# bee-hive/MedGP

Hardware: AMD Instinct MI355X
Metric: per-patient nlml+grad evals/sec at D=24 N=512 (higher is better)
Workload: dtype f64; 1 GPU; config 4 shard: 512 patients/GPU x N=512, D=24, Q=5, R=8, H=1114, LMC-SM + hier-gamma prior, nlml+grad; patients_per_gpu=512, cohort=512, N=512, D=24, Q=5, R=8, H=1114, parallelism=patient-sharded x1 (no collective)

## Files before the change

medgp_amd/csrc/kernels_wgrad.h:

```cpp
#pragma once
#include "medgp_dev.h"
#include "kernels_assemble.h"

#define WG_KC 32
#define WG_THREADS 256
#ifndef WG_MINWAVES
#define WG_MINWAVES 3
#endif

#define WG_CHUNK_MFMA(ac, buf) \
    _Pragma("unroll") for (int h = 0; h < 4; h++) \
        _Pragma("unroll") for (int ct = 0; ct < 4; ct++) { \
            if (ct > ctmax) continue;    \
            const v2d bf = *(const v2d *)&Bs[buf][16 * ct + li][8 * h + 2 * g]; \
            _Pragma("unroll") for (int s = 0; s < 2; s++) acc[ct] = __builtin_amdgcn_mfma_f64_16x16x4f64(ac[h][s], bf[s], acc[ct], 0, 0, 0); \
        }

template <int QT, int Q0 = 0, int PF = 1>
__global__ void __launch_bounds__(WG_THREADS, WG_MINWAVES) k_wgrad(MedgpDev L, int nbatch, int ntiles, int nbp) {
    __shared__ __attribute__((aligned(16))) double smem[2 * 64 * (WG_KC + 2)];
    typedef double (*BsT)[64][WG_KC + 2];
    BsT Bs = (BsT)smem;
    double (*Ws)[66] = (double (*)[66])smem;
    __shared__ __attribute__((aligned(16))) double rowc[4][16][2 + 2 * QT];

    int b, tix;
    if (nbatch >= 64) {
        const int xcd = blockIdx.x & 7, rest = blockIdx.x >> 3;
        b = (rest / ntiles) * 8 + xcd;
        tix = rest % ntiles;
    } else {
        int x = blockIdx.x;
        const int total = nbp * ntiles;
        if (x >= total) return;
        if (PF > 1 && total <= 1024 && ((x >> 8) & 1)) {
            const int v0 = x & ~255, m = min(256, total - v0);
            x = v0 + (m - 1 - (x & 255));
        }
        b = x % nbp;
        tix = x / nbp;
    }
    if (b >= nbatch) return;
    if (L.status[b] < 0) return;
    const int slot = __builtin_amdgcn_readfirstlane(L.bslot[b]);
    const int n = __builtin_amdgcn_readfirstlane(L.pn[slot]);
    const int ld = L.ldn, npad = medgp_roundup(n, 64), nb = npad / 64;
    int I, J;
    tile_decode(tix, I, J);
    if (I >= nb) return;
    const int tid = threadIdx.x, lane = tid & 63, li = lane & 15, g = lane >> 4;
    const int w = __builtin_amdgcn_readfirstlane(tid >> 6);
    const double *U = L.Linv + (size_t)b * ld * ld;

#ifdef MEDGP_STAMPS
    unsigned long long wst[4] = {0, 0, 0, 0}, wlast;
    asm volatile("s_memtime %0\n\ts_waitcnt lgkmcnt(0)" : "=s"(wlast)::"memory");
#define WSTAMP(k) do { unsigned long long t_; asm volatile("s_memtime %0\n\ts_waitcnt lgkmcnt(0)" : "=s"(t_)::"memory"); wst[k] += t_ - wlast; wlast = t_; } while (0)
#else
#define WSTAMP(k) do {} while (0)
#endif
    v4d acc[4];
#pragma unroll
    for (int ct = 0; ct < 4; ct++) acc[ct] = (v4d){0.0, 0.0, 0.0, 0.0};
    {
        const int k0 = 64 * I, nch = (npad - k0) / WG_KC;
        const int ctmax = (I == J) ? w : 3;
        const double *Arow = U + (size_t)(64 * I + 16 * w + li) * ld + k0 + 2 * g;
        const int srow = tid >> 2, scg = (tid & 3) * 8;
        const double *Bsrc = U + (size_t)(64 * J + srow) * ld + k0 + scg;
        if constexpr (PF == 1) {
            v2d bst[4], an[4];
#pragma unroll
            for (int u = 0; u < 4; u++) bst[u] = *(const v2d *)(Bsrc + 2 * u);
#pragma unroll
            for (int h = 0; h < 4; h++) an[h] = *(const v2d *)(Arow + 8 * h);
#pragma unroll
            for (int u = 0; u < 4; u++) *(v2d *)&Bs[0][srow][scg + 2 * u] = bst[u];
            __syncthreads();
            for (int c = 0; c < nch; c++) {
                const int buf = c & 1;
                v2d ac[4];
#pragma unroll
                for (int h = 0; h < 4; h++) ac[h] = an[h];
                if (c + 1 < nch) {
#pragma unroll
                    for (int u = 0; u < 4; u++) bst[u] = *(const v2d *)(Bsrc + (c + 1) * WG_KC + 2 * u);
#pragma unroll
                    for (int h = 0; h < 4; h++) an[h] = *(const v2d *)(Arow + (c + 1) * WG_KC + 8 * h);
                }
                WG_CHUNK_MFMA(ac, buf);
                if (c + 1 < nch) {
#pragma unroll
                    for (int u = 0; u < 4; u++) *(v2d *)&Bs[buf ^ 1][srow][scg + 2 * u] = bst[u];
                }
                __syncthreads();
            }
        } else {
            v2d bst[PF][4], an[PF][4];
#pragma unroll
            for (int st = 0; st < PF; st++)
                if (st < nch) {
#pragma unroll
                    for (int u = 0; u < 4; u++) bst[st][u] = *(const v2d *)(Bsrc + st * WG_KC + 2 * u);
#pragma unroll
                    for (int h = 0; h < 4; h++) an[st][h] = *(const v2d *)(Arow + st * WG_KC + 8 * h);
                }
#pragma unroll
            for (int u = 0; u < 4; u++) *(v2d *)&Bs[0][srow][scg + 2 * u] = bst[0][u];
            __syncthreads();
            for (int c0 = 0; c0 < nch; c0 += PF) {
#pragma unroll
                for (int st = 0; st < PF; st++) {
                    const int c = c0 + st;
                    if (c >= nch) break;
                    v2d ac[4];
#pragma unroll
                    for (int h = 0; h < 4; h++) ac[h] = an[st][h];
                    if (c + PF < nch) {
#pragma unroll
                        for (int u = 0; u < 4; u++) bst[st][u] = *(const v2d *)(Bsrc + (c + PF) * WG_KC + 2 * u);
#pragma unroll
                        for (int h = 0; h < 4; h++) an[st][h] = *(const v2d *)(Arow + (c + PF) * WG_KC + 8 * h);
                    }
                    WG_CHUNK_MFMA(ac, (st & 1));
                    if (c + 1 < nch) {
#pragma unroll
                        for (int u = 0; u < 4; u++) *(v2d *)&Bs[(st + 1) & 1][srow][scg + 2 * u] = bst[(st + 1) % PF][u];
                    }
                    __syncthreads();
                }
            }
        }
    }
    WSTAMP(0);
#pragma unroll
    for (int ct = 0; ct < 4; ct++)
#pragma unroll
        for (int r = 0; r < 4; r++) Ws[16 * w + 4 * r + g][16 * ct + li] = acc[ct][r];
    __syncthreads();

    WSTAMP(1);
    const double *hyp = L.hyp + (size_t)b * L.hyp_stride;
    const double *t = L.pt + (size_t)slot * L.pld;
    const int *meta = L.pmeta + (size_t)slot * L.pld;
    const double *alpha = L.alpha + (size_t)b * ld;
    const int *seg = L.pseg + (size_t)slot * (L.D + 1);
    const int *roff = L.proff + (size_t)slot * (L.D + 1), *coff = L.pcoff + (size_t)slot * (L.D + 1);
    const double *csb = L.cs + ((size_t)b * L.Q + Q0) * ld, *snb = L.sn + ((size_t)b * L.Q + Q0) * ld;
    double *slab = L.slab + (size_t)b * L.slab_stride;
    const int Qall = L.Q;
    const int Rmax = L.slab_R, Cmax = L.slab_C;

    double wq[QT], cq[QT];
#pragma unroll
    for (int q = 0; q < QT; q++) { wq[q] = hyp[hyp_off_w(L) + Q0 + q]; cq[q] = hyp[hyp_off_c(L) + Q0 + q]; }
    double cq2n[QT];
#pragma unroll
    for (int q = 0; q < QT; q++) cq2n[q] = uniform_d(-cq[q] * MEDGP_LOG2E);
    const int j = 64 * J + lane;
    const bool jv = j < n;
    const double tj = t[j], aj = alpha[j];
    const int mj = jv ? meta[j] : -1;
    double csj[QT], snj[QT];
#pragma unroll
    for (int q = 0; q < QT; q++) { csj[q] = csb[q * ld + j]; snj[q] = snb[q * ld + j]; }
    const int mprev = __shfl_up(mj, 1);
    const bool leader = (lane == 0) || (mj != mprev);
    const unsigned long long lmask = __ballot(leader);
    int segend;
    {
        unsigned long long above = (lane == 63) ? 0ull : (lmask >> (lane + 1));
        segend = above ? (lane + 1 + __builtin_ctzll(above)) : 64;
    }
    const unsigned long long upto = lmask & ((lane == 63) ? ~0ull : ((2ull << lane) - 1ull));
    const int segstart = 63 - __builtin_clzll(upto);
    const bool seglast = (lane == segend - 1);
    const int cslot = (mj >= 0) ? coff[mj] + (J - seg[mj] / 64) : 0;
    const int rg = 4 * I + w;

    double sS[QT], sM[QT], sV[QT];
#pragma unroll
    for (int q = 0; q < QT; q++) { sS[q] = 0.0; sM[q] = 0.0; sV[q] = 0.0; }
    int mcur = -2;
    const int irow = 64 * I + 16 * w + (lane & 15);
    const double r_t = t[irow], r_a = alpha[irow];
    const int r_m = (irow < n) ? meta[irow] : -1;
    double r_cs[QT], r_sn[QT];
#pragma unroll
    for (int q = 0; q < QT; q++) { r_cs[q] = csb[q * ld + irow]; r_sn[q] = snb[q * ld + irow]; }
    if (lane < 16) {
        rowc[w][lane][0] = r_t; rowc[w][lane][1] = r_a;
#pragma unroll
        for (int q = 0; q < QT; q++) { rowc[w][lane][2 + 2 * q] = r_cs[q]; rowc[w][lane][3 + 2 * q] = r_sn[q]; }
    }
    __builtin_amdgcn_wave_barrier();
    for (int rr = 0; rr <= 16; rr++) {
        const int i = 64 * I + 16 * w + rr;
        int mi = -1;
        if (rr < 16) mi = __builtin_amdgcn_readlane(r_m, rr);
        if (mi != mcur) {
            if (mcur >= 0) {
                const int rslot = roff[mcur] + (rg - seg[mcur] / 16);
                double fv[3 * QT];
#pragma unroll
                for (int q = 0; q < QT; q++) { fv[q] = sS[q]; fv[QT + q] = -wq[q] * sM[q]; fv[2 * QT + q] = -2.0 * cq[q] * sV[q]; }
#pragma unroll
                for (int dlt = 1; dlt < 64; dlt <<= 1) {
                    double up[3 * QT];
#pragma unroll
                    for (int k = 0; k < 3 * QT; k++) up[k] = __shfl_up(fv[k], dlt);
                    if (lane - dlt >= segstart) {
#pragma unroll
                        for (int k = 0; k < 3 * QT; k++) fv[k] += up[k];
                    }
                }
                if (seglast && mj >= 0) {
#pragma unroll
                    for (int k = 0; k < 3 * QT; k++) slab[((size_t)((k / QT) * Qall + Q0 + (k % QT)) * Rmax + rslot) * Cmax + cslot] = fv[k];
                }
            }
#pragma unroll
            for (int q = 0; q < QT; q++) { sS[q] = 0.0; sM[q] = 0.0; sV[q] = 0.0; }
            mcur = mi;
        }
        if (rr == 16 || mi < 0) continue;
        const v2d ta = *(const v2d *)&rowc[w][rr][0];
        const double ti = ta[0], ai = ta[1];
        double wv = Ws[16 * w + rr][lane] - ai * aj;
        if (I == J && j == i) L.wdiag[(size_t)b * ld + i] = wv;
        const bool valid = jv && (j <= i);
        wv = valid ? ((mi == mj && j < i) ? 2.0 * wv : wv) : 0.0;
        const double dt = ti - tj, dd = dt * dt;
#pragma unroll
        for (int q = 0; q < QT; q++) {
            const v2d csn = *(const v2d *)&rowc[w][rr][2 + 2 * q];
            const double ci = csn[0], si = csn[1];
            const double we = wv * exp2_nonpos(cq2n[q] * dd);
            const double cd = ci * csj[q] + si * snj[q];
            const double sd = si * csj[q] - ci * snj[q];
            const double p = we * cd;
            sS[q] += p;
            sM[q] += (we * sd) * dt;
            sV[q] += p * dd;
        }
    }
    WSTAMP(2);
#ifdef MEDGP_STAMPS
    if (lane == 0 && b < 64) {
        unsigned long long *dbg = (unsigned long long *)(L.xk + (size_t)b * 64 * 64);
        for (int e = 0; e < 3; e++) atomicAdd(&dbg[e], wst[e]);
        atomicAdd(&dbg[3], 1ull);
    }
#endif
}
```

medgp_amd/csrc/medgp_capi.hip:

```cpp
#include "../../include/medgp_hip.h"
#include "medgp_dev.h"
#include "kernels_core.h"
#include "kernels_v0.h"
#include "kernels_cholinv.h"
#include "kernels_cholinv_la.h"
#include "kernels_assemble.h"
#include "kernels_wgrad.h"
#include "kernels_io.h"
#include "kernels_cohort.h"

#include <algorithm>
#include <chrono>
#include <cmath>
#include <cstdarg>
#include <cstdio>
#include <cstdlib>
#include <cstring>
#include <string>
#include <vector>

namespace {

enum KernelId { KID_PREP = 0, KID_ASSEMBLE, KID_CHOLINV, KID_LA_STEP, KID_LA_AUX, KID_LAUUM, KID_GRADBINS, KID_WGRAD, KID_EPILOGUE, KID_PREDICT, KID_COUNT };
const char *const kKernelNames[KID_COUNT] = {"k_prep", "k_assemble", "k_cholinv", "k_la_step", "k_la_aux", "k_lauum", "k_gradbins", "k_wgrad", "k_epilogue", "k_predict"};
// ... 554 lines not shown
#endif
        if (route == ROUTE_WG44) hipLaunchKernelGGL((k_cholinv<4, 4, 0>), dim3(nbatch), dim3(256), 0, stream, L, want_mode);
        else hipLaunchKernelGGL((k_cholinv<8, 4, 0>), dim3(nbatch), dim3(512), 0, stream, L, want_mode);
    }
    int from_slab = 0;
#ifdef MEDGP_STAMPS
    if (getenv("MEDGP_DBG_NOWGRAD")) { HIPCHK(c, hipGetLastError()); return MEDGP_OK; }
#endif
    if (flag_grad) {
        const int wg_tiles = tri(nt64);
        const int nbp = (ragged && nbatch < 64) ? (nbatch | 1) : nbatch;
        const dim3 tg(std::max(8 * ((nbatch + 7) / 8), nbp) * wg_tiles), tb(WG_THREADS);
        from_slab = 1;
        Launcher lw(c, KID_WGRAD, stream);
        const int pf = c->wgrad_deep >= 0 ? c->wgrad_deep : ((long)nbatch * wg_tiles <= 16L * c->num_cu ? 2 : 1);
#define MEDGP_WGL(QQ, Q0) do { if (pf >= 2) hipLaunchKernelGGL((k_wgrad<QQ, Q0, 2>), tg, tb, 0, stream, L, nbatch, wg_tiles, nbp); \
                               else hipLaunchKernelGGL((k_wgrad<QQ, Q0, 1>), tg, tb, 0, stream, L, nbatch, wg_tiles, nbp); } while (0)
#define MEDGP_WG1(QQ) case QQ: MEDGP_WGL(QQ, 0); break;
#define MEDGP_WG2(QR) case 8 + QR: MEDGP_WGL(8, 0); MEDGP_WGL(QR, 8); break;
        switch (c->use_v0 ? 0 : L.Q) {
        MEDGP_WG1(1) MEDGP_WG1(2) MEDGP_WG1(3) MEDGP_WG1(4) MEDGP_WG1(5) MEDGP_WG1(6) MEDGP_WG1(7) MEDGP_WG1(8)
        MEDGP_WG2(1) MEDGP_WG2(2) MEDGP_WG2(3) MEDGP_WG2(4) MEDGP_WG2(5) MEDGP_WG2(6) MEDGP_WG2(7) MEDGP_WG2(8)
#undef MEDGP_WG1
#undef MEDGP_WG2
#undef MEDGP_WGL
        default: from_slab = 0; break;
        }
        if (!from_slab) lw.kid = -1;
        lw.finish();
        if (!from_slab) {
            { Launcher l(c, KID_LAUUM, stream); hipLaunchKernelGGL(k_lauum_v0, dim3(tri(nt64), nbatch), dim3(256), 0, stream, L); }
            const int nbins = L.Q * tri(L.D);
            { Launcher l(c, KID_GRADBINS, stream); hipLaunchKernelGGL(k_gradbins_v0, dim3((nbins + 255) / 256, nbatch), dim3(256), 0, stream, L); }
        }
    }
    if (flag_grad && from_slab) {
        const int nbins3 = 3 * L.Q * tri(L.D);
        Launcher l(c, KID_EPILOGUE, stream);
        hipLaunchKernelGGL(k_slabsum, dim3(nbatch, (nbins3 + 255) / 256), dim3(256), 0, stream, L);
    }
    if (nlml_dev) {
        Launcher l(c, KID_EPILOGUE, stream);
        const int nparts = (2 * nbatch >= c->num_cu) ? 1 : std::min(MEDGP_EPI_PARTS, (L.H + 255) / 256);
        hipLaunchKernelGGL(k_epilogue, dim3(nbatch, nparts), dim3(256), 0, stream, L, theta_dev, flag_grad, from_slab, nlml_dev, grad_dev, (int *)status_dev);
    }
    HIPCHK(c, hipGetLastError());
    return MEDGP_OK;
}


void choose_routes(const medgp_ctx *c, BatchPlan &P, std::vector<LaNeed> &las, std::vector<int> &la_of) {
    long long S = 0;
    for (const SizeClass &k : P.cls) S += k.tsum;
    las.clear();
    la_of.assign(P.cls.size(), -1);
    for (size_t i = 0; i < P.cls.size(); i++) {
        SizeClass &k = P.cls[i];
        bool la = false;
        if (!c->use_v0 && !c->pin_route && k.nbmax >= 2) {
            if (c->force_mc > 0) la = true;
            else if (c->force_mc == 0 && k.nbmax >= 3 && !c->no_classes) la = wg_cost(k.nbmax) * c->num_cu * (k.nbmax <= 4 ? 7 : 9) >= 16 * S;
            else if (c->force_mc == 0 && k.nbmax >= 3) la = k.count <= (c->num_cu * (k.nbmax <= 4 ? 7 : 9)) / 16;
        }
        if (la) {
            k.route = ROUTE_LA;
            S -= k.tsum;
            la_of[i] = (int)las.size();
            las.push_back({k.count, k.nbmax, k.ld, LaArgs{}});
        } else {
            const int shape = c->pin_route ? 84 : (c->cholinv_nw ? c->cholinv_nw : ((k.count > c->num_cu || k.nbmax <= 4) ? 44 : 84));
            k.route = shape == 44 ? ROUTE_WG44 : ROUTE_WG84;
        }
    }
}

void la_needs(const BatchPlan &P, const std::vector<LaNeed> &las, const std::vector<int> &la_of, size_t *part, size_t *small) {
    std::vector<size_t> wp(P.nwaves, 0), ws(P.nwaves, 0);
    for (size_t i = 0; i < P.cls.size(); i++)
        if (la_of[i] >= 0) { wp[P.cls[i].wave] += la_part_doubles(las[la_of[i]], P.with_u); ws[P.cls[i].wave] += la_small_doubles(las[la_of[i]]); }
    *part = *small = 0;
    for (int w = 0; w < P.nwaves; w++) { *part = std::max(*part, wp[w]); *small = std::max(*small, ws[w]); }
}

size_t screen_chunk_end(const medgp_ctx *c, const std::vector<int> &ns, int ninit, size_t e0, size_t total, int max_entries) {
    size_t e = e0, bytes = 0;
    long long work = 0;
    while (e < total && (int)(e - e0) < max_entries) {
        const int nb = blocks64(ns[e / ninit]);
        const size_t ldb = (size_t)64 << size_bucket(nb), per = 8 * ldb * ldb;
        if (e > e0 && bytes + per > c->screen_budget) break;
        if (e > e0 && nb >= 45 && work >= c->screen_work) break;
        bytes += per; work += (long long)nb * nb; e++;
    }
    return e;
}

struct ScreenChunk { size_t e0, e1; };
struct ScreenCut {
    std::vector<ScreenChunk> chunks;
    bool two = false;
    int lane_rows = 0;
    size_t cap_mat = 0, cap_vec = 0, cap_tab = 0, cap_part = 0, cap_small = 0;
};
void screen_cut(const medgp_ctx *c, const std::vector<int> &walk_n, int ninit, ScreenCut &S) {
    const size_t total = walk_n.size() * (size_t)ninit;
    S.two = c->screen_lanes >= 2 && c->max_batch >= 2 && screen_chunk_end(c, walk_n, ninit, 0, total, c->max_batch) < total;
    S.lane_rows = S.two ? c->max_batch / 2 : c->max_batch;
    S.chunks.clear();
    for (size_t e0 = 0; e0 < total;) { const size_t e = screen_chunk_end(c, walk_n, ninit, e0, total, S.lane_rows); S.chunks.push_back({e0, e}); e0 = e; }
    BatchPlan P;
    std::vector<LaNeed> las;
    std::vector<int> la_of, en;
    int lf = -1, ll = -1;
    size_t lc = 0;
    for (const ScreenChunk &ch : S.chunks) {
        const int nf = walk_n[ch.e0 / ninit], nl = walk_n[(ch.e1 - 1) / ninit];
        if (nf == nl && nf == lf && nl == ll && ch.e1 - ch.e0 == lc) continue;
        en.resize(ch.e1 - ch.e0);
        for (size_t x = ch.e0; x < ch.e1; x++) en[x - ch.e0] = walk_n[x / ninit];
        layout_plan(c, en.data(), (int)en.size(), false, P);
        choose_routes(c, P, las, la_of);
        size_t lp = 0, ls = 0;
        la_needs(P, las, la_of, &lp, &ls);
        S.cap_mat = std::max(S.cap_mat, P.need_mat); S.cap_vec = std::max(S.cap_vec, P.need_vec); S.cap_tab = std::max(S.cap_tab, P.need_tab);
        S.cap_part = std::max(S.cap_part, lp); S.cap_small = std::max(S.cap_small, ls);
        lf = nf; ll = nl; lc = ch.e1 - ch.e0;
    }
}

int run_pipeline(medgp_ctx *c, int nbatch, int max_n, const double *theta_dev, int flag_grad, bool need_inverse, int min_n,
                 double *nlml_dev, double *grad_dev, int32_t *status_dev, bool store_ukk = false, bool persist = false,
                 BatchPlan *Pp = nullptr, hipStream_t st_main = nullptr, int aux0 = 0, int naux = kAuxStreams, hipEvent_t ev_fork_in = nullptr) {
    (void)max_n; (void)nbatch;
    BatchPlan &P = Pp ? *Pp : c->plan;
    if (!st_main) st_main = c->stream;
    hipEvent_t ev_fork = ev_fork_in ? ev_fork_in : c->ev_fork;
    const bool forms_u = flag_grad || need_inverse || store_ukk;
    if (forms_u && !P.with_u) return fail(c, MEDGP_ERR_ARG, "internal: plan laid out without Linv for a call that forms it");
    if (persist && P.nwaves > 1)
        return fail(c, MEDGP_ERR_CAPACITY, "the call's per-entry matrices exceed the memory budget of %zu GB (MEDGP_MEM_BUDGET_GB) and its outputs need all of them at once: split the call",
                    c->mem_budget >> 30);
    { int rc = ensure_arena(c, P.mat0 + P.need_mat, P.with_u ? P.mat0 + P.need_mat : 0, P.vec0 + P.need_vec, P.tab0 + P.need_tab, P.need_slab); if (rc) return rc; }
    c->last_has_inverse = (flag_grad || need_inverse) && P.nwaves == 1;
    std::vector<LaNeed> las;
    std::vector<int> la_of;
    choose_routes(c, P, las, la_of);
    const int nstr = std::max(0, std::min(c->class_streams, naux));
    for (int w = 0; w < P.nwaves; w++) {
        size_t i0 = 0, i1;
        while (i0 < P.cls.size() && P.cls[i0].wave != w) i0++;
        i1 = i0;
        while (i1 < P.cls.size() && P.cls[i1].wave == w) i1++;
        std::vector<LaNeed> wl;
        std::vector<int> wl_of(P.cls.size(), -1);
        for (size_t i = i0; i < i1; i++) if (la_of[i] >= 0) { wl_of[i] = (int)wl.size(); wl.push_back(las[la_of[i]]); }
        if (!wl.empty()) { int rc = ensure_la(c, wl, P.with_u, P.la_part0, P.la_small0); if (rc) return rc; }
        const bool fork = i1 - i0 > 1 && nstr > 0 && c->aux[aux0];
        if (fork) HIPCHK(c, hipEventRecord(ev_fork, st_main));
        bool used[kAuxStreams] = {false, false, false, false};
        for (size_t i = i0; i < i1; i++) {
            const SizeClass &k = P.cls[i];
            hipStream_t st = st_main;
            int ai = -1;
            if (fork && i > i0) {
                ai = aux0 + (int)((i - i0 - 1) % nstr);
                st = c->aux[ai];
                if (!used[ai]) { HIPCHK(c, hipStreamWaitEvent(st, ev_fork, 0)); used[ai] = true; }
            }
            const MedgpDev V = class_view(c, P, k);
            int rc = run_pipeline_one(c, st, V, k.count, k.nbmax, theta_dev, flag_grad, need_inverse, min_n, nlml_dev, grad_dev, status_dev, store_ukk,
                                      P.en.data() + k.b0, k.route, wl_of[i] >= 0 ? &wl[wl_of[i]].A : nullptr);
            if (rc) return rc;
        }
        if (fork)
            for (int ai = aux0; ai < aux0 + nstr; ai++)
                if (used[ai]) {
                    HIPCHK(c, hipEventRecord(c->ev_join[ai], c->aux[ai]));
                    HIPCHK(c, hipStreamWaitEvent(st_main, c->ev_join[ai], 0));
                }
    }
    return MEDGP_OK;
}

}

extern "C" {

int medgp_abi_version(void) { return 3; }

int medgp_device_count(void) {
    int n = 0;
    if (hipGetDeviceCount(&n) != hipSuccess) return 0;
    return n;
}

const char *medgp_last_error(const medgp_ctx *ctx) { return ctx ? ctx->err.c_str() : g_create_error.c_str(); }

int medgp_create(medgp_ctx **out, int device, int kernel_index, int Q, int D, int R) {
    if (!out) return fail(nullptr, MEDGP_ERR_ARG, "out is NULL");
    *out = nullptr;
    if (kernel_index == MEDGP_KERNEL_SE) { Q = 1; D = 1; R = 0; }
    if (kernel_index == MEDGP_KERNEL_SM) { D = 1; R = 0; }
    int nc = num_cov(kernel_index, Q, D, R);
    if (nc < 0) return fail(nullptr, MEDGP_ERR_ARG, "unsupported kernel_index %d (supported: 0 SE, 7 LMC-SM, 8 SM)", kernel_index);
    if (Q < 1 || D < 1 || R < 0) return fail(nullptr, MEDGP_ERR_ARG, "bad Q/D/R = %d/%d/%d", Q, D, R);
    if (D > MEDGP_MAX_D) return fail(nullptr, MEDGP_ERR_ARG, "D = %d exceeds the supported %d outputs", D, MEDGP_MAX_D);
    int ndev = medgp_device_count();
    if (ndev <= 0) return fail(nullptr, MEDGP_ERR_NODEVICE, "no HIP device visible; libmedgp_hip has no CPU fallback");
    if (device < 0 || device >= ndev) return fail(nullptr, MEDGP_ERR_ARG, "device %d outside [0, %d)", device, ndev);
    medgp_ctx *c = new medgp_ctx();
    c->device = device;
    c->kidx = kernel_index; c->Q = Q; c->D = D; c->R = R;
    c->nlik = (kernel_index == MEDGP_KERNEL_LMC_SM) ? D : 1;
    c->H = c->nlik + nc;
    if (hipSetDevice(device) != hipSuccess || hipStreamCreateWithFlags(&c->own_stream, hipStreamNonBlocking) != hipSuccess) {
        delete c;
        return fail(nullptr, MEDGP_ERR_HIP, "cannot initialise device %d", device);
    }
    c->stream = c->own_stream;
    { const char *e = getenv("MEDGP_CHOLINV_NW"); c->cholinv_nw = e ? atoi(e) : 0; }
    { const char *e = getenv("MEDGP_LA_PARK"); if (e) c->la_park = atoi(e); }
    { const char *e = getenv("MEDGP_LA_PARK_MAXBATCH"); if (e) c->la_park_maxbatch = atoi(e); }
    { const char *e = getenv("MEDGP_MULTI_CU"); c->force_mc = e ? atoi(e) : 0; }
    { const char *e = getenv("MEDGP_CLASS_STREAMS"); if (e) c->class_streams = std::max(0, std::min(kAuxStreams, atoi(e))); }
    { const char *e = getenv("MEDGP_NO_CLASSES"); c->no_classes = e ? atoi(e) : 0; }
    { const char *e = getenv("MEDGP_WGRAD_DEEP"); c->wgrad_deep = e ? std::max(1, atoi(e)) : -1; }
    { const char *e = getenv("MEDGP_DEBUG_FAIL_ATTEMPTS"); c->dbg_fail = e ? atoi(e) : 0; }
    { const char *e = getenv("MEDGP_MEM_BUDGET_GB"); if (e && atof(e) > 0) c->mem_budget = (size_t)(atof(e) * 1073741824.0); }
    { const char *e = getenv("MEDGP_SCREEN_LANES"); if (e && atoi(e) >= 1) c->screen_lanes = std::min(2, atoi(e)); }
    { const char *e = getenv("MEDGP_SCREEN_WORK"); if (e && atoll(e) > 0) c->screen_work = atoll(e); }
    { const char *e = getenv("MEDGP_SCREEN_BUDGET_GB"); if (e && atof(e) > 0) c->screen_budget = (size_t)(atof(e) * 1073741824.0); }
    for (int i = 0; i < kAuxStreams; i++) {
        (void)hipStreamCreateWithFlags(&c->aux[i], hipStreamNonBlocking);
        (void)hipEventCreateWithFlags(&c->ev_join[i], hipEventDisableTiming);
    }
    (void)hipEventCreateWithFlags(&c->ev_fork, hipEventDisableTiming);
    (void)hipStreamCreateWithFlags(&c->s_screen1, hipStreamNonBlocking);
    for (hipEvent_t *e : {&c->ev_fork1, &c->ev_screen0}) (void)hipEventCreateWithFlags(e, hipEventDisableTiming);
    { hipDeviceProp_t pr; if (hipGetDeviceProperties(&pr, device) == hipSuccess) c->num_cu = pr.multiProcessorCount; }
    *out = c;
    return MEDGP_OK;
}

void medgp_destroy(medgp_ctx *c) {
    if (!c) return;
    (void)hipSetDevice(c->device);
    (void)hipStreamSynchronize(c->stream);
    for (auto &e : c->events) { (void)hipEventDestroy(e.a); (void)hipEventDestroy(e.b); }
    for (hipEvent_t e : c->ev_pool) (void)hipEventDestroy(e);
    free_all(c);
    for (int i = 0; i < kAuxStreams; i++) {
        if (c->aux[i]) { (void)hipStreamSynchronize(c->aux[i]); (void)hipStreamDestroy(c->aux[i]); }
        if (c->ev_join[i]) (void)hipEventDestroy(c->ev_join[i]);
    }
    if (c->ev_fork) (void)hipEventDestroy(c->ev_fork);
    if (c->s_screen1) { (void)hipStreamSynchronize(c->s_screen1); (void)hipStreamDestroy(c->s_screen1); }
    for (hipEvent_t e : {c->ev_fork1, c->ev_screen0}) if (e) (void)hipEventDestroy(e);
    if (c->h_screen_tab) (void)hipHostFree(c->h_screen_tab);
    for (hipStream_t st : {c->s_up, c->s_down}) if (st) { (void)hipStreamSynchronize(st); (void)hipStreamDestroy(st); }
    for (int i = 0; i < 2; i++) { if (c->ev_up[i]) (void)hipEventDestroy(c->ev_up[i]); if (c->ev_k[i]) (void)hipEventDestroy(c->ev_k[i]); }
    if (c->ev_stage) (void)hipEventDestroy(c->ev_stage);
    if (c->h_stage) (void)hipHostFree(c->h_stage);
    if (c->h_bounce) (void)hipHostFree(c->h_bounce);
    if (c->h_small) (void)hipHostFree(c->h_small);
    if (c->d_small) (void)hipFree(c->d_small);
    for (int i = 0; i < 2; i++) {
        if (c->pin_buf[i]) (void)hipHostFree(c->pin_buf[i]);
        if (c->pin_ev[i]) (void)hipEventDestroy(c->pin_ev[i]);
        if (c->ev_lane[i]) (void)hipEventDestroy(c->ev_lane[i]);
    }
    if (c->own_stream) (void)hipStreamDestroy(c->own_stream);
    delete c;
}

int medgp_num_hyp(const medgp_ctx *c) { return c ? c->H : MEDGP_ERR_ARG; }

int medgp_set_pi(medgp_ctx *c, double pi) {
    if (!c || !(pi > 0)) return MEDGP_ERR_ARG;
    c->pi = pi;
    c->dev.pi = pi;
    return MEDGP_OK;
}

int medgp_set_stream(medgp_ctx *c, void *s) {
    if (!c) return MEDGP_ERR_ARG;
    HIPCHK(c, hipSetDevice(c->device));
    HIPCHK(c, hipStreamSynchronize(c->stream));
    c->stream = s ? (hipStream_t)s : c->own_stream;
    return MEDGP_OK;
}

int medgp_synchronize(medgp_ctx *c) {
    if (!c) return MEDGP_ERR_ARG;
    HIPCHK(c, hipSetDevice(c->device));
    HIPCHK(c, hipStreamSynchronize(c->stream));
    if (c->s_down) HIPCHK(c, hipStreamSynchronize(c->s_down));
    free_retired(c);
    return MEDGP_OK;
}

int medgp_reserve(medgp_ctx *c, int max_slots, int max_n, int max_batch) {
    if (!c) return MEDGP_ERR_ARG;
    if (max_slots < 1 || max_n < 1 || max_batch < 1) return fail(c, MEDGP_ERR_ARG, "medgp_reserve: non-positive capacity");
    HIPCHK(c, hipSetDevice(c->device));
    HIPCHK(c, hipStreamSynchronize(c->stream));
    free_all(c);
    c->max_slots = max_slots; c->max_n = max_n; c->max_batch = max_batch;
    const int ldn = medgp_roundup(max_n, 64);
    c->ldn = ldn;
    const size_t S = max_slots, B = max_batch, Q = c->Q, D = c->D, H = c->H;
    int rc;
    if ((rc = dalloc(c, &c->d_pn, 2 * S))) return rc;
    if ((rc = dalloc(c, &c->d_pt, 2 * S * ldn))) return rc;
    if ((rc = dalloc(c, &c->d_py, 2 * S * ldn))) return rc;
    if ((rc = dalloc(c, &c->d_pmeta, 2 * S * ldn))) return rc;
    if ((rc = dalloc(c, &c->d_pseg, 2 * S * (D + 1)))) return rc;
    if ((rc = dalloc(c, &c->d_proff, 2 * S * (D + 1)))) return rc;
    if ((rc = dalloc(c, &c->d_pcoff, 2 * S * (D + 1)))) return rc;
    if ((rc = dalloc(c, &c->d_one_slot, 1))) return rc;
    if ((rc = dalloc(c, &c->d_prior, S * H))) return rc;
    if ((rc = dalloc(c, &c->d_prior_on, S))) return rc;
    if ((rc = dalloc(c, &c->d_bslot, B))) return rc;
    if ((rc = dalloc(c, &c->d_bpos, B))) return rc;
    if ((rc = dalloc(c, &c->d_tpos, B))) return rc;
    c->d_screen_theta = nullptr; c->screen_theta_cap = 0; c->tpos_on = false;
    if ((rc = dalloc(c, &c->d_status, B))) return rc;
    if ((rc = dalloc(c, &c->d_jit, B))) return rc;
    if ((rc = dalloc(c, &c->d_bn, B))) return rc;
    if ((rc = dalloc(c, &c->d_theta, B * H))) return rc;
    if ((rc = dalloc(c, &c->d_nlml, B))) return rc;
    if ((rc = dalloc(c, &c->d_grad, B * H))) return rc;
    if ((rc = dalloc(c, &c->d_status_out, B))) return rc;
    if ((rc = dalloc(c, &c->d_theta1, B * H))) return rc;
    if ((rc = dalloc(c, &c->d_nlml1, B))) return rc;
    if ((rc = dalloc(c, &c->d_grad1, B * H))) return rc;
    if ((rc = dalloc(c, &c->d_status1, B))) return rc;
    c->lane_pending[0] = c->lane_pending[1] = false;
    c->d_prior_stage = nullptr; c->d_prior_slots = nullptr; c->prior_stage_rows = 0;
    MedgpDev &L = c->dev;
    L.kidx = c->kidx; L.Q = c->Q; L.D = c->D; L.R = c->R; L.H = c->H; L.nlik = c->nlik;
    L.ldn = ldn; L.pld = ldn; L.max_slots = max_slots; L.max_batch = max_batch;
    L.bpos = nullptr;
    L.tpos = nullptr;
    L.hyp_stride = (int)(D + Q * D * D + 2 * Q);
    L.pi = c->pi;
    L.dbg_fail = c->dbg_fail;
    double *hyp, *scal, *Sb, *SMb, *SVb;
    L.slab_R = ldn / 16 + (int)D;
    L.slab_C = ldn / 64 + (int)D;
    L.slab_stride = (size_t)3 * Q * L.slab_R * L.slab_C;
    c->full_mat = B * ldn * ldn; c->full_vec = B * ldn; c->full_tab = B * Q * ldn; c->full_slab = B * L.slab_stride;
    L.Kmat = L.Linv = L.z = L.alpha = L.wdiag = L.cs = L.sn = L.slab = nullptr;
    {
        size_t fr = 0, tot = 0;
        if (hipMemGetInfo(&fr, &tot) == hipSuccess && fr > 0) {
            c->mem_budget = std::min(c->mem_budget, fr / 10 * 7);
            c->screen_budget = std::min(c->screen_budget, c->mem_budget);
        }
    }
    if (2 * c->full_mat * sizeof(double) <= kArenaEager) rc = ensure_arena(c, c->full_mat, c->full_mat, c->full_vec, c->full_tab, c->full_slab, true);
    else rc = ensure_arena(c, 0, 0, 0, 0, 0, true);
    if (rc) return rc;
    double *xk;
    if ((rc = dalloc(c, &xk, B * 64 * 64))) return rc;
    L.xk = xk; L.jit = c->d_jit; L.bn = c->d_bn;
    if ((rc = dalloc(c, &hyp, B * L.hyp_stride))) return rc;
    if ((rc = dalloc(c, &scal, B * 4))) return rc;
    if ((rc = dalloc(c, &L.epi_lp, B * MEDGP_EPI_PARTS))) return rc;
    if ((rc = dalloc(c, &L.epi_ticket, B))) return rc;
    HIPCHK(c, hipMemsetAsync(L.epi_ticket, 0, B * sizeof(int), c->stream));
    if ((rc = dalloc(c, &Sb, B * Q * D * D))) return rc;
    if ((rc = dalloc(c, &SMb, B * Q * D * D))) return rc;
    if ((rc = dalloc(c, &SVb, B * Q * D * D))) return rc;
    L.pn = c->d_pn; L.pt = c->d_pt; L.py = c->d_py; L.pmeta = c->d_pmeta; L.pseg = c->d_pseg;
    L.proff = c->d_proff; L.pcoff = c->d_pcoff;
    L.prior = c->d_prior; L.prior_on = c->d_prior_on; L.bslot = c->d_bslot;
    L.hyp = hyp; L.scal = scal;
    L.status = c->d_status; L.S = Sb; L.SM = SMb; L.SV = SVb;
    HIPCHK(c, hipMemsetAsync(c->d_prior_on, 0, S, c->stream));
    HIPCHK(c, hipMemsetAsync(c->d_pn, 0, 2 * S * sizeof(int), c->stream));
    HIPCHK(c, hipStreamSynchronize(c->stream));
    c->h_n.assign(max_slots, -1);
    c->h_perm.assign(max_slots, {});
    c->h_perm_identity.assign(max_slots, 1);
    c->h_bslot.assign(max_batch, -1);
    c->last_nbatch = 0;
    c->plan = BatchPlan{};
    c->last_has_inverse = false;
    c->pred_cap = 0;
    c->d_stage = nullptr;
    if (c->h_stage) { (void)hipHostFree(c->h_stage); c->h_stage = nullptr; }
    c->stage_cap = 0;
    c->stage_pending = false;
    return MEDGP_OK;
}

int medgp_reserve_plan(medgp_ctx *c, int count, const int32_t *n, int ninit) {
    if (!c) return MEDGP_ERR_ARG;
    if (c->max_slots == 0) return fail(c, MEDGP_ERR_CAPACITY, "call medgp_reserve first");
    if (count < 1 || !n || ninit < 0) return fail(c, MEDGP_ERR_ARG, "medgp_reserve_plan: bad argument");
    for (int i = 0; i < count; i++)
        if (n[i] < 0 || n[i] > c->max_n) return fail(c, MEDGP_ERR_CAPACITY, "medgp_reserve_plan: n[%d] = %d outside [0, %d]", i, n[i], c->max_n);
    HIPCHK(c, hipSetDevice(c->device));
    std::vector<int> ns(n, n + count);
    std::stable_sort(ns.begin(), ns.end(), [](int a, int b) { return a > b; });
    size_t nk = 0, nu = 0, nvec = 0, ntab = 0, nslab = 0, npart = 0, nsmall = 0;
    BatchPlan P;
    std::vector<LaNeed> las;
    std::vector<int> la_of;
    auto take = [&](const int *en, int nb, bool with_u) {
        layout_plan(c, en, nb, with_u, P);
        choose_routes(c, P, las, la_of);
        size_t lp = 0, ls = 0;
        la_needs(P, las, la_of, &lp, &ls);
        nk = std::max(nk, P.need_mat); if (with_u) nu = std::max(nu, P.need_mat);
        nvec = std::max(nvec, P.need_vec); ntab = std::max(ntab, P.need_tab); nslab = std::max(nslab, P.need_slab);
        npart = std::max(npart, lp); nsmall = std::max(nsmall, ls);
    };
    take(ns.data(), std::min(count, c->max_batch), true);
    if (ninit > 0) {
        ScreenCut SC;
        screen_cut(c, ns, ninit, SC);
        const size_t f = SC.two ? 2 : 1;
        nk = std::max(nk, f * SC.cap_mat); nvec = std::max(nvec, f * SC.cap_vec); ntab = std::max(ntab, f * SC.cap_tab);
        npart = std::max(npart, f * SC.cap_part); nsmall = std::max(nsmall, f * SC.cap_small);
    }
    int rc;
    if ((rc = ensure_arena(c, nk, nu, nvec, ntab, nslab, true))) return rc;
    if (npart && (rc = arena_ensure(c, AR_LA_PART, npart * sizeof(double), 0, true, nullptr))) return rc;
    if (nsmall && (rc = arena_ensure(c, AR_LA_SMALL, nsmall * sizeof(double), 0, true, nullptr))) return rc;
    if (!c->retired.empty()) { if ((rc = sync_ctx_streams(c))) return rc; free_retired(c); }
    return MEDGP_OK;
}

int medgp_alloc_stats(const medgp_ctx *c, double *seconds, int64_t *calls, int64_t *arena_bytes) {
    if (!c) return MEDGP_ERR_ARG;
    if (seconds) *seconds = c->alloc_s;
    if (calls) *calls = c->alloc_calls;
    if (arena_bytes) { int64_t b = 0; for (int i = 0; i < AR_COUNT; i++) b += (int64_t)c->arena[i].bytes; *arena_bytes = b; }
    return MEDGP_OK;
}

namespace {
struct UpEntry { int slot, n; const int32_t *meta; const float *t, *y; };

inline size_t up_payload_bytes(int n, int D) { return ((size_t)n * 20 + (size_t)(D + 1) * 12 + 7) & ~(size_t)7; }

int upload_patients(medgp_ctx *c, const std::vector<UpEntry> &ents) {
    const int D = c->D, S = c->max_slots, ldn = c->ldn;
    const bool use_meta = (c->kidx == MEDGP_KERNEL_LMC_SM);
    std::vector<uint8_t> seen(ents.size() > 1 ? (size_t)S : 0, 0);
    for (const UpEntry &e : ents) {
        if (e.slot < 0 || e.slot >= S) return fail(c, MEDGP_ERR_CAPACITY, "slot %d outside [0, %d)", e.slot, S);
        if (!seen.empty()) {
            if (seen[e.slot]) return fail(c, MEDGP_ERR_ARG, "slot %d appears twice in one packed upload", e.slot);
            seen[e.slot] = 1;
        }
        if (e.n < 0 || e.n > c->max_n) return fail(c, MEDGP_ERR_CAPACITY, "n = %d outside [0, %d]", e.n, c->max_n);
        if (e.n > 0 && (!e.t || !e.y)) return fail(c, MEDGP_ERR_ARG, "t / y is NULL");
        if (use_meta && e.n > 0 && !e.meta) return fail(c, MEDGP_ERR_ARG, "meta is NULL for the multi-output kernel");
        if (use_meta)
            for (int i = 0; i < e.n; i++)
                if (e.meta[i] < 0 || e.meta[i] >= D) return fail(c, MEDGP_ERR_ARG, "meta[%d] = %d outside [0, %d)", i, e.meta[i], D);
    }
    size_t bytes = 0;
    for (const UpEntry &e : ents) bytes += 2 * (sizeof(MedgpUpHdr) + up_payload_bytes(e.n, D));
    HIPCHK(c, hipSetDevice(c->device));
    if (c->stage_pending) { HIPCHK(c, hipEventSynchronize(c->ev_stage)); c->stage_pending = false; }
    if (bytes > c->stage_cap) {
        const size_t cap = std::max<size_t>(bytes + bytes / 4, 1 << 16);
        if (c->h_stage) (void)hipHostFree(c->h_stage);
        c->h_stage = nullptr;
        HIPCHK(c, hipHostMalloc((void **)&c->h_stage, cap, hipHostMallocDefault));
        HIPCHK(c, hipStreamSynchronize(c->stream));
        if (c->d_stage) {
            (void)hipFree(c->d_stage);
            c->allocs.erase(std::remove(c->allocs.begin(), c->allocs.end(), (void *)c->d_stage), c->allocs.end());
            c->d_stage = nullptr;
        }
        int rc = dalloc(c, &c->d_stage, cap);
        if (rc) return rc;
        c->stage_cap = cap;
    }
    if (!c->ev_stage) HIPCHK(c, hipEventCreateWithFlags(&c->ev_stage, hipEventDisableTiming));
    std::vector<std::vector<int>> perms(ents.size());
    std::vector<uint8_t> ident(ents.size(), 1);
    int nent = 0;
    for (size_t k = 0; k < ents.size(); k++) {
        const UpEntry &e = ents[k];
        std::vector<int> &perm = perms[k];
        perm.resize(e.n);
        if (use_meta) {
            std::vector<int> pos(D + 1, 0);
            for (int i = 0; i < e.n; i++) pos[e.meta[i] + 1]++;
            for (int d = 0; d < D; d++) pos[d + 1] += pos[d];
            for (int i = 0; i < e.n; i++) perm[pos[e.meta[i]]++] = i;
        } else {
            for (int i = 0; i < e.n; i++) perm[i] = i;
        }
        for (int i = 0; i < e.n; i++) if (perm[i] != i) { ident[k] = 0; break; }
        nent += ident[k] ? 1 : 2;
    }
    MedgpUpHdr *hdr = (MedgpUpHdr *)c->h_stage;
    size_t off = (size_t)nent * sizeof(MedgpUpHdr);
    int ie = 0;
    auto pack = [&](const UpEntry &e, int dev_slot, const int *perm) {
        hdr[ie].slot = dev_slot; hdr[ie].n = e.n; hdr[ie].off = (long long)off; ie++;
        double *pt = (double *)(c->h_stage + off), *py = pt + e.n;
        int *pm = (int *)(py + e.n), *seg = pm + e.n, *roff = seg + (D + 1), *coff = roff + (D + 1);
        for (int i = 0; i < e.n; i++) {
            const int src = perm ? perm[i] : i;
            pt[i] = (double)e.t[src];
            py[i] = (double)e.y[src];
            pm[i] = use_meta ? e.meta[src] : 0;
        }
        for (int d = 0; d <= D; d++) seg[d] = roff[d] = coff[d] = 0;
        if (perm || !use_meta) {
            if (use_meta) { for (int i = 0; i < e.n; i++) seg[pm[i] + 1]++; for (int d = 0; d < D; d++) seg[d + 1] += seg[d]; }
            else seg[1] = e.n;
            for (int d = 0; d < D; d++) {
                const int a = seg[d], z = seg[d + 1];
                roff[d + 1] = roff[d] + (z > a ? (z - 1) / 16 - a / 16 + 1 : 0);
                coff[d + 1] = coff[d] + (z > a ? (z - 1) / 64 - a / 64 + 1 : 0);
            }
        }
        off += up_payload_bytes(e.n, D);
    };
    for (size_t k = 0; k < ents.size(); k++) {
        pack(ents[k], ents[k].slot, perms[k].data());
        if (!ident[k]) pack(ents[k], ents[k].slot + S, nullptr);
    }
    HIPCHK(c, hipMemcpyAsync(c->d_stage, c->h_stage, off, hipMemcpyHostToDevice, c->stream));
    HIPCHK(c, hipEventRecord(c->ev_stage, c->stream));
    c->stage_pending = true;
    hipLaunchKernelGGL(k_scatter_patients, dim3(nent), dim3(256), 0, c->stream, (const char *)c->d_stage, D, ldn, c->d_pn, c->d_pt,
                       c->d_py, c->d_pmeta, c->d_pseg, c->d_proff, c->d_pcoff);
    HIPCHK(c, hipGetLastError());
    for (size_t k = 0; k < ents.size(); k++) {
        const int s = ents[k].slot;
        c->h_n[s] = ents[k].n;
        c->h_perm[s] = std::move(perms[k]);
        c->h_perm_identity[s] = ident[k];
    }
    c->last_nbatch = 0;
    c->last_has_inverse = false;
    return MEDGP_OK;
}
}

int medgp_set_patient(medgp_ctx *c, int slot, int n, const int32_t *meta, const float *t, const float *y) {
    if (!c) return MEDGP_ERR_ARG;
    if (c->max_slots == 0) return fail(c, MEDGP_ERR_CAPACITY, "call medgp_reserve first");
    return upload_patients(c, {UpEntry{slot, n, meta, t, y}});
}

int medgp_set_patients(medgp_ctx *c, int nslots, const int32_t *slots, const int64_t *offsets, const int32_t *meta,
                       const float *t, const float *y) {
    if (!c) return MEDGP_ERR_ARG;
    if (c->max_slots == 0) return fail(c, MEDGP_ERR_CAPACITY, "call medgp_reserve first");
    if (nslots < 1 || !slots || !offsets) return fail(c, MEDGP_ERR_ARG, "medgp_set_patients: bad argument");
    std::vector<UpEntry> ents(nslots);
    for (int k = 0; k < nslots; k++) {
        const int64_t a = offsets[k], z = offsets[k + 1];
        if (a < 0 || z < a || z - a > c->max_n) return fail(c, MEDGP_ERR_CAPACITY, "offsets[%d..%d] = %lld..%lld: bad length", k, k + 1, (long long)a, (long long)z);
        ents[k] = UpEntry{slots[k], (int)(z - a), meta ? meta + a : nullptr, t ? t + a : nullptr, y ? y + a : nullptr};
    }
    return upload_patients(c, ents);
}

namespace {
int upload_priors(medgp_ctx *c, int nrows, const int32_t *slots, const uint8_t *flag, const int32_t *type, const uint8_t *is_exp,
                  const float *p0, const float *p1) {
    const int H = c->H;
    if (flag && (!type || !is_exp || !p0 || !p1)) return fail(c, MEDGP_ERR_ARG, "prior arrays must all be given");
    std::vector<uint8_t> seen((slots && nrows > 1) ? (size_t)c->max_slots : 0, 0);
    for (int k = 0; slots && k < nrows; k++) {
        if (slots[k] < 0 || slots[k] >= c->max_slots) return fail(c, MEDGP_ERR_CAPACITY, "slot %d outside [0, %d)", slots[k], c->max_slots);
        if (!seen.empty()) {
            if (seen[slots[k]]) return fail(c, MEDGP_ERR_ARG, "slot %d appears twice in one medgp_set_priors", slots[k]);
            seen[slots[k]] = 1;
        }
    }
    if (flag)
        for (size_t h = 0; h < (size_t)nrows * H; h++)
            if (type[h] < -1 || type[h] > 2) return fail(c, MEDGP_ERR_ARG, "prior type[%zu] = %d unsupported (KDE prior type 3 is never constructed by the reference's mains)", h, type[h]);
    HIPCHK(c, hipSetDevice(c->device));
    if ((size_t)nrows > c->prior_stage_rows) {
        { int rcs = sync_ctx_streams(c); if (rcs) return rcs; }
        for (void *q : {(void *)c->d_prior_stage, (void *)c->d_prior_slots})
            if (q) { (void)hipFree(q); c->allocs.erase(std::remove(c->allocs.begin(), c->allocs.end(), q), c->allocs.end()); }
        c->d_prior_stage = nullptr; c->d_prior_slots = nullptr; c->prior_stage_rows = 0;
        const size_t rows = std::max<size_t>(nrows, 16);
        int rc;
        if ((rc = dalloc(c, &c->d_prior_stage, rows * H))) return rc;
        if ((rc = dalloc(c, &c->d_prior_slots, rows))) return rc;
        c->prior_stage_rows = rows;
    }
    const size_t row_bytes = sizeof(MedgpPrior) * (size_t)H, slot_bytes = ((sizeof(int) * (size_t)nrows) + 15) & ~(size_t)15;
    void *pin = nullptr;
    int rc = pin_stage(c, slot_bytes + row_bytes * nrows, &pin);
    if (rc) return rc;
    int *hs = (int *)pin;
    MedgpPrior *hp = (MedgpPrior *)((char *)pin + slot_bytes);
    for (int k = 0; k < nrows; k++) {
        hs[k] = slots ? slots[k] : -1;
        for (int h = 0; h < H; h++) {
// ... 609 lines not shown
```

Measured before the change: 192,300 evals/s.

## Use buffer loads in wgrad GEMM, skip zero triangle chunks, specialize off-diagonal tiles

Replaces the pointer-based global loads of the inverse-Cholesky tiles with buffer-resource loads that use a scalar base plus per-lane offsets, which cuts address arithmetic and VGPR use. On diagonal tiles the first two K-chunks skip MFMAs over the zero upper-triangular part of Linv. A compile-time specialization for off-diagonal tiles drops the ctmax guard and the per-element validity and doubling logic, moving the factor of two into the segment flush. A capacity check is added so one matrix stays under the 32-bit buffer range.

```diff
diff --git a/medgp_amd/csrc/kernels_wgrad.h b/medgp_amd/csrc/kernels_wgrad.h
--- a/medgp_amd/csrc/kernels_wgrad.h
+++ b/medgp_amd/csrc/kernels_wgrad.h
@@ -1,6 +1,8 @@
 #pragma once
 #include "medgp_dev.h"
 #include "kernels_assemble.h"
+#include "kernels_cholinv.h"
+#include <type_traits>
 
 #define WG_KC 32
 #define WG_THREADS 256
@@ -8,13 +10,18 @@
 #define WG_MINWAVES 3
 #endif
 
-#define WG_CHUNK_MFMA(ac, buf) \
-    _Pragma("unroll") for (int h = 0; h < 4; h++) \
+#define WG_CHUNK_MFMA(ac, buf, hlo) \
+    _Pragma("unroll") for (int h = 0; h < 4; h++) { \
+        if (h < (hlo)) continue; \
         _Pragma("unroll") for (int ct = 0; ct < 4; ct++) { \
             if (ct > ctmax) continue;    \
             const v2d bf = *(const v2d *)&Bs[buf][16 * ct + li][8 * h + 2 * g]; \
             _Pragma("unroll") for (int s = 0; s < 2; s++) acc[ct] = __builtin_amdgcn_mfma_f64_16x16x4f64(ac[h][s], bf[s], acc[ct], 0, 0, 0); \
-        }
+        } \
+    }
+#define WG_LOADA(dst, c) _Pragma("unroll") for (int h = 0; h < 4; h++) (dst)[h] = ci_bload(rsU, voA, soA + (c) * (WG_KC * 8) + 64 * h)
+#define WG_LOADB(dst, c) _Pragma("unroll") for (int u = 0; u < 4; u++) (dst)[u] = ci_bload(rsU, voB, soB + (c) * (WG_KC * 8) + 16 * u)
+#define WG_STAGE(buf, src) _Pragma("unroll") for (int u = 0; u < 4; u++) *(v2d *)&Bs[buf][srow][scg + 2 * u] = (src)[u]
 
 template <int QT, int Q0 = 0, int PF = 1>
 __global__ void __launch_bounds__(WG_THREADS, WG_MINWAVES) k_wgrad(MedgpDev L, int nbatch, int ntiles, int nbp) {
@@ -64,35 +71,48 @@
     for (int ct = 0; ct < 4; ct++) acc[ct] = (v4d){0.0, 0.0, 0.0, 0.0};
     {
         const int k0 = 64 * I, nch = (npad - k0) / WG_KC;
-        const int ctmax = (I == J) ? w : 3;
-        const double *Arow = U + (size_t)(64 * I + 16 * w + li) * ld + k0 + 2 * g;
         const int srow = tid >> 2, scg = (tid & 3) * 8;
-        const double *Bsrc = U + (size_t)(64 * J + srow) * ld + k0 + scg;
+        const unsigned uld = (unsigned)ld, mat_bytes = uld * uld * 8u;
+        __amdgpu_buffer_rsrc_t rsU;
+        {
+            const unsigned long long ub = (unsigned long long)U;
+            const unsigned lo32 = __builtin_amdgcn_readfirstlane((unsigned)ub), hi32 = __builtin_amdgcn_readfirstlane((unsigned)(ub >> 32));
+            rsU = __builtin_amdgcn_make_buffer_rsrc((void *)(((unsigned long long)hi32 << 32) | lo32), 0, (int)mat_bytes, 0x00020000);
+        }
+        const int voA = (int)(((unsigned)li * uld + 2u * g) * 8u), voB = (int)(((unsigned)srow * uld + (unsigned)scg) * 8u);
+        const int soA = __builtin_amdgcn_readfirstlane((int)(((unsigned)(64 * I + 16 * w) * uld + (unsigned)k0) * 8u));
+        const int soB = __builtin_amdgcn_readfirstlane((int)(((unsigned)(64 * J) * uld + (unsigned)k0) * 8u));
+        auto phase1 = [&](auto full_tag) {
+        const int ctmax = decltype(full_tag)::value ? 3 : ((I == J) ? w : 3);
         if constexpr (PF == 1) {
             v2d bst[4], an[4];
-#pragma unroll
-            for (int u = 0; u < 4; u++) bst[u] = *(const v2d *)(Bsrc + 2 * u);
-#pragma unroll
-            for (int h = 0; h < 4; h++) an[h] = *(const v2d *)(Arow + 8 * h);
-#pragma unroll
-            for (int u = 0; u < 4; u++) *(v2d *)&Bs[0][srow][scg + 2 * u] = bst[u];
+            WG_LOADB(bst, 0);
+            WG_LOADA(an, 0);
+            WG_STAGE(0, bst);
             __syncthreads();
-            for (int c = 0; c < nch; c++) {
+#pragma unroll
+            for (int c = 0; c < 2; c++) {
+                v2d ac[4];
+#pragma unroll
+                for (int h = 0; h < 4; h++) ac[h] = an[h];
+                const int cn = min(c + 1, nch - 1);
+                WG_LOADB(bst, cn);
+                WG_LOADA(an, cn);
+                WG_CHUNK_MFMA(ac, c, 2 * w - 4 * c);
+                WG_STAGE(c ^ 1, bst);
+                __syncthreads();
+            }
+            for (int c = 2; c < nch; c++) {
                 const int buf = c & 1;
                 v2d ac[4];
 #pragma unroll
                 for (int h = 0; h < 4; h++) ac[h] = an[h];
                 if (c + 1 < nch) {
-#pragma unroll
-                    for (int u = 0; u < 4; u++) bst[u] = *(const v2d *)(Bsrc + (c + 1) * WG_KC + 2 * u);
-#pragma unroll
-                    for (int h = 0; h < 4; h++) an[h] = *(const v2d *)(Arow + (c + 1) * WG_KC + 8 * h);
-                }
-                WG_CHUNK_MFMA(ac, buf);
-                if (c + 1 < nch) {
-#pragma unroll
-                    for (int u = 0; u < 4; u++) *(v2d *)&Bs[buf ^ 1][srow][scg + 2 * u] = bst[u];
-                }
+                    WG_LOADB(bst, c + 1);
+                    WG_LOADA(an, c + 1);
+                }
+                WG_CHUNK_MFMA(ac, buf, 0);
+                if (c + 1 < nch) WG_STAGE(buf ^ 1, bst);
                 __syncthreads();
             }
         } else {
@@ -100,13 +120,10 @@
 #pragma unroll
             for (int st = 0; st < PF; st++)
                 if (st < nch) {
-#pragma unroll
-                    for (int u = 0; u < 4; u++) bst[st][u] = *(const v2d *)(Bsrc + st * WG_KC + 2 * u);
-#pragma unroll
-                    for (int h = 0; h < 4; h++) an[st][h] = *(const v2d *)(Arow + st * WG_KC + 8 * h);
-                }
-#pragma unroll
-            for (int u = 0; u < 4; u++) *(v2d *)&Bs[0][srow][scg + 2 * u] = bst[0][u];
+                    WG_LOADB(bst[st], st);
+                    WG_LOADA(an[st], st);
+                }
+            WG_STAGE(0, bst[0]);
             __syncthreads();
             for (int c0 = 0; c0 < nch; c0 += PF) {
 #pragma unroll
@@ -117,20 +134,18 @@
 #pragma unroll
                     for (int h = 0; h < 4; h++) ac[h] = an[st][h];
                     if (c + PF < nch) {
-#pragma unroll
-                        for (int u = 0; u < 4; u++) bst[st][u] = *(const v2d *)(Bsrc + (c + PF) * WG_KC + 2 * u);
-#pragma unroll
-                        for (int h = 0; h < 4; h++) an[st][h] = *(const v2d *)(Arow + (c + PF) * WG_KC + 8 * h);
+                        WG_LOADB(bst[st], c + PF);
+                        WG_LOADA(an[st], c + PF);
                     }
-                    WG_CHUNK_MFMA(ac, (st & 1));
-                    if (c + 1 < nch) {
-#pragma unroll
-                        for (int u = 0; u < 4; u++) *(v2d *)&Bs[(st + 1) & 1][srow][scg + 2 * u] = bst[(st + 1) % PF][u];
-                    }
+                    WG_CHUNK_MFMA(ac, (st & 1), 2 * w - 4 * c);
+                    if (c + 1 < nch) WG_STAGE((st + 1) & 1, bst[(st + 1) % PF]);
                     __syncthreads();
                 }
             }
         }
+        };
+        if (PF == 1 && I != J) phase1(std::true_type{});
+        else phase1(std::false_type{});
     }
     WSTAMP(0);
 #pragma unroll
@@ -194,6 +209,7 @@
         for (int q = 0; q < QT; q++) { rowc[w][lane][2 + 2 * q] = r_cs[q]; rowc[w][lane][3 + 2 * q] = r_sn[q]; }
     }
     __builtin_amdgcn_wave_barrier();
+    const bool diagt = I == J;
     for (int rr = 0; rr <= 16; rr++) {
         const int i = 64 * I + 16 * w + rr;
         int mi = -1;
@@ -201,6 +217,11 @@
         if (mi != mcur) {
             if (mcur >= 0) {
                 const int rslot = roff[mcur] + (rg - seg[mcur] / 16);
+                if (!diagt) {
+                    const double fac = (mcur == mj) ? 2.0 : 1.0;
+#pragma unroll
+                    for (int q = 0; q < QT; q++) { sS[q] *= fac; sM[q] *= fac; sV[q] *= fac; }
+                }
                 double fv[3 * QT];
 #pragma unroll
                 for (int q = 0; q < QT; q++) { fv[q] = sS[q]; fv[QT + q] = -wq[q] * sM[q]; fv[2 * QT + q] = -2.0 * cq[q] * sV[q]; }
@@ -208,15 +229,15 @@
                 for (int dlt = 1; dlt < 64; dlt <<= 1) {
                     double up[3 * QT];
 #pragma unroll
-                    for (int k = 0; k < 3 * QT; k++) up[k] = __shfl_up(fv[k], dlt);
+                    for (int e = 0; e < 3 * QT; e++) up[e] = __shfl_up(fv[e], dlt);
                     if (lane - dlt >= segstart) {
 #pragma unroll
-                        for (int k = 0; k < 3 * QT; k++) fv[k] += up[k];
+                        for (int e = 0; e < 3 * QT; e++) fv[e] += up[e];
                     }
                 }
                 if (seglast && mj >= 0) {
 #pragma unroll
-                    for (int k = 0; k < 3 * QT; k++) slab[((size_t)((k / QT) * Qall + Q0 + (k % QT)) * Rmax + rslot) * Cmax + cslot] = fv[k];
+                    for (int e = 0; e < 3 * QT; e++) slab[((size_t)((e / QT) * Qall + Q0 + (e % QT)) * Rmax + rslot) * Cmax + cslot] = fv[e];
                 }
             }
 #pragma unroll
@@ -227,9 +248,11 @@
         const v2d ta = *(const v2d *)&rowc[w][rr][0];
         const double ti = ta[0], ai = ta[1];
         double wv = Ws[16 * w + rr][lane] - ai * aj;
-        if (I == J && j == i) L.wdiag[(size_t)b * ld + i] = wv;
-        const bool valid = jv && (j <= i);
-        wv = valid ? ((mi == mj && j < i) ? 2.0 * wv : wv) : 0.0;
+        if (diagt) {
+            if (j == i) L.wdiag[(size_t)b * ld + i] = wv;
+            const bool valid = jv && (j <= i);
+            wv = valid ? ((mi == mj && j < i) ? 2.0 * wv : wv) : 0.0;
+        }
         const double dt = ti - tj, dd = dt * dt;
 #pragma unroll
         for (int q = 0; q < QT; q++) {
diff --git a/medgp_amd/csrc/medgp_capi.hip b/medgp_amd/csrc/medgp_capi.hip
--- a/medgp_amd/csrc/medgp_capi.hip
+++ b/medgp_amd/csrc/medgp_capi.hip
@@ -880,6 +880,8 @@
 int medgp_reserve(medgp_ctx *c, int max_slots, int max_n, int max_batch) {
     if (!c) return MEDGP_ERR_ARG;
     if (max_slots < 1 || max_n < 1 || max_batch < 1) return fail(c, MEDGP_ERR_ARG, "medgp_reserve: non-positive capacity");
+    if ((size_t)medgp_roundup(max_n, 64) * medgp_roundup(max_n, 64) * sizeof(double) > 0xffffffffull)
+        return fail(c, MEDGP_ERR_ARG, "medgp_reserve: max_n above 23168 (one matrix must stay below 4 GiB)");
     HIPCHK(c, hipSetDevice(c->device));
     HIPCHK(c, hipStreamSynchronize(c->stream));
     free_all(c);
```

Measured after the change: 195,600 evals/s (median of 6 runs). +1.7%, better.
